# Rhizomatica/mercury

Measured on AMD Instinct MI355X. Metric: RX frames/s (mode 8, max 50 LDPC iters), higher is better.
Workload: dtype f64

## Files before the change

### include/mercury_gpu.h

```cpp
#ifndef MERCURY_GPU_H
#define MERCURY_GPU_H

#include <stddef.h>
#include <stdint.h>

#ifdef __cplusplus
extern "C" {
#endif

#define MGPU_OK 0
#define MGPU_ERR_ARG 1
#define MGPU_ERR_DEVICE 2
#define MGPU_ERR_TABLES 3
#define MGPU_ERR_UNSUPPORTED 4

#define MGPU_DEC_GBF 0
#define MGPU_DEC_SPA 1
#define MGPU_DEC_MINSUM 2
#define MGPU_DEC_SPA_FAST 3

#define MGPU_EST_ZF 0
#define MGPU_EST_LS 1

typedef struct mgpu_ctx mgpu_ctx;
// ... 129 lines not shown
    double avg_iterations;
    long long crc_ok_frames;
} mgpu_error_rate;
int mgpu_baseband_test_esn0(mgpu_ctx* ctx, const double* esn0_db, int npoints, long long frames_per_point, uint64_t seed, uint64_t frame0,
                            int channel, mgpu_error_rate* out);

int mgpu_passband_to_baseband(mgpu_ctx* ctx, const double* passband , int W, int in_size,
                              const double* carrier_hz , int filter, const int* start , int count,
                              int decimation, double* out_c128 );
int mgpu_time_sync_preamble(mgpu_ctx* ctx, const double* baseband_interp_c128 , int W, int size, int step,
                            int location_to_return, int nTrials_max, int* delay , double* correlation );
int mgpu_freq_sync(mgpu_ctx* ctx, const double* baseband_c128 , int W, int stride, double* freq_offset_hz );
int mgpu_time_sync_mfsk(mgpu_ctx* ctx, const double* baseband_interp_c128 , int W, int size, int search_start_symb,
                        int* delay );
int mgpu_detect_ack_pattern(mgpu_ctx* ctx, const double* baseband_interp_c128 , int W, int size, int pattern,
                            double* metric , int* matched );
int mgpu_detect_ack_pattern_from_passband(mgpu_ctx* ctx, const double* passband , int W, int size, double carrier_hz,
                                          int pattern, double* metric , int* matched );
int mgpu_last_sync_kernel_ms(mgpu_ctx* ctx, float* ms);

int mgpu_enable_timing(mgpu_ctx* ctx, int on);
int mgpu_kernel_ms_avg(mgpu_ctx* ctx, float ms[2], int* n_launches);
int mgpu_decoder_hard_frames(mgpu_ctx* ctx, long long* frames);
int mgpu_host_path_last(mgpu_ctx* ctx, int* chunk_frames, int* n_chunks, float* fill_ms, float* drain_ms, float* total_ms);
int mgpu_last_kernel_ms(mgpu_ctx* ctx, float ms[2]);

int mgpu_debug_mfsk_sync(mgpu_ctx* ctx, const double* energy, int W, int nslots, int size, const int* search_start, int variant, int* delay);
int mgpu_debug_p2b_variant(int variant);
int mgpu_debug_span_energy(mgpu_ctx* ctx, const double* bb, int W, int size, const int* wv, const int* off, int n, int len, int variant, double* sum,
                           int* cnt);
int mgpu_debug_spa_math(mgpu_ctx* ctx, const double* in, int n, double* tanh_out, double* atanh_out);
int mgpu_debug_select_peak(mgpu_ctx* ctx, const double* cand_vals, int n, int ncand_max, const int* ncand, const int* size, const int* loc, int step,
                           int nTrials_max, int* delay, double* corr);

int mgpu_debug_occupancy(mgpu_ctx* ctx, int which);

int mgpu_debug_tsync_metric(mgpu_ctx* ctx, const double* baseband_interp, int W, int size, int step, int variant, const int* start, const int* sub_size,
                            double* vals);

int mgpu_debug_glibc_trig(mgpu_ctx* ctx, const double* in, int n, double* atan_out, double* sin_out, double* cos_out);

#ifdef __cplusplus
}
#endif
#endif
```

### mercury_amd/csrc/api.hip

```cpp
#include <hip/hip_runtime.h>

#include <cstdio>
#include <cstdlib>
#include <cstring>
#include <fstream>
#include <algorithm>
#include <atomic>
#include <functional>
#include <stdexcept>
#include <string>
#include <vector>

#include "ctx.hpp"
#include "numa.hpp"

typedef void (*fe_kernel_t)(MgpuDev, const double*, int, float*, float*, float*, double*, MgpuTapsDev);
static fe_kernel_t fe_kernel(int threads) { return threads == 1024 ? mgpu_frontend_kernel_t1024 : mgpu_frontend_kernel; }

thread_local std::string g_create_error;

namespace mgpu_detail {

void ctx_alloc(mgpu_ctx* c) {
    const auto& t = c->tab;
// ... 82 lines not shown
        std::vector<uint8_t> msg(size_t(full > 0 ? full : 1), 0);
        const uint16_t zero = mgpu::crc16_modbus(msg.data(), full);
        std::vector<uint16_t> tab(size_t(full > 0 ? full : 1) * 8, 0);
        for (int b = 0; b < full; ++b)
            for (int j = 0; j < 8; ++j) {
                msg[b] = uint8_t(1u << j);
                tab[size_t(b) * 8 + j] = uint16_t(mgpu::crc16_modbus(msg.data(), full) ^ zero);
                msg[b] = 0;
            }
        l.crc_tab = c->keep(upload(tab));
        l.crc_init = zero;
    }
    l.gdesc = c->keep(upload(t.graph.gdesc));
    l.gkpack = c->keep(upload(t.graph.gkpack));
    l.vinfo_g = c->keep(upload(t.graph.vinfo_g));
    l.Sg = t.graph.Sg;
    l.sadr = c->keep(upload(t.graph.sadr));
    l.bhead = c->keep(upload(t.graph.bhead));
    l.bmask = c->keep(upload(t.graph.bmask));
    l.vinfo2 = c->keep(upload(t.graph.vinfo2));
    l.DM = t.graph.DM;
    l.S = d.S; l.N = d.N; l.P = d.P; l.K = d.K; l.E = d.E; l.nReal = d.nReal; l.payload_stride = d.payload_stride;
    l.max_iters = d.max_iters; l.minsum_alpha = d.minsum_alpha;
    l.hard_frames = reinterpret_cast<unsigned long long*>(c->keep(upload(std::vector<uint64_t>(64, 0))));
    {
        int w[4] = {100, 230, 45, 150};
        if (const char* e = getenv("MERCURY_SPA_SPEC_WEIGHT")) {
            const int n = sscanf(e, "%d,%d,%d,%d", &w[0], &w[1], &w[2], &w[3]);
            if (n == 1) { w[1] = w[2] = w[3] = w[0]; }
            else if (n == 2) { w[2] = w[0]; w[3] = w[1]; }
            else if (n == 3) { w[3] = w[2]; }
        }
        const int nbins = d.S / 64 > 0 ? d.S / 64 : 1;
        auto sample_min = [&](int weight) {
            const long long m = (static_cast<long long>(weight) * 16 + nbins - 1) / nbins;
            return weight <= 0 ? 0 : (m > 0x7fffff ? 0x7fffff : int(m));
        };
        auto byte = [&](int weight) { const int m = sample_min(weight); return unsigned(m > 255 ? 255 : m); };
        l.spec_sample_pack = byte(w[0]) | byte(w[1]) << 8 | byte(w[2]) << 16 | byte(w[3]) << 24;
    }
    HIPCK(hipStreamCreate(&c->stream));
    for (auto& q : c->ev) for (auto& e : q) HIPCK(hipEventCreate(&e));
    for (auto& e : c->sync_ev) HIPCK(hipEventCreate(&e));

    const bool mfsk = t.mfsk_M > 0;
    {
        const char* e = getenv("MERCURY_FE_THREADS");
// ... 8 lines not shown
    {
        int geo[6];
        mgpu_tsync_fine_geometry(geo);
        HIPCK(hipFuncSetAttribute(reinterpret_cast<const void*>(mgpu_tsync_metric_fine_kernel_r4), hipFuncAttributeMaxDynamicSharedMemorySize, geo[2]));
        HIPCK(hipFuncSetAttribute(reinterpret_cast<const void*>(mgpu_tsync_metric_fine_kernel_r8), hipFuncAttributeMaxDynamicSharedMemorySize, geo[5]));
    }
    switch (c->cfg.decoder) {
        case MGPU_DEC_SPA:
            if (!t.graph.fp64_limit.empty()) throw std::runtime_error(t.graph.fp64_limit);
            c->lds_dec = mgpu_spa_lds_bytes(d.S, d.N);
            {
                const int ne = std::max(4, (d.S + 1023) / 1024);
                if (ne > 8) throw std::runtime_error("graph too large for the sum-product kernel");
                if (t.graph.maxdeg > mgpu_spa_max_degree(ne)) throw std::runtime_error("check degree exceeds the sum-product kernel's unrolled product walk");
                switch (ne) {
                    case 4: c->spa_kernel = mgpu_ldpc_spa_kernel_ne4; break;
                    case 5: c->spa_kernel = mgpu_ldpc_spa_kernel_ne5; break;
                    case 6: c->spa_kernel = mgpu_ldpc_spa_kernel_ne6; break;
                    case 7: c->spa_kernel = mgpu_ldpc_spa_kernel_ne7; break;
                    default: c->spa_kernel = mgpu_ldpc_spa_kernel_ne8; break;
                }
            }
            HIPCK(hipFuncSetAttribute(reinterpret_cast<const void*>(c->spa_kernel), hipFuncAttributeMaxDynamicSharedMemorySize, int(c->lds_dec)));
            break;
        case MGPU_DEC_GBF:
            c->lds_dec = mgpu_gbf_lds_bytes(d.N);
            HIPCK(hipFuncSetAttribute(reinterpret_cast<const void*>(mgpu_ldpc_gbf_kernel), hipFuncAttributeMaxDynamicSharedMemorySize, int(c->lds_dec)));
            break;
        case MGPU_DEC_MINSUM: {
            if (!t.graph.fp32_limit.empty()) throw std::runtime_error(t.graph.fp32_limit);
            c->lds_dec = mgpu_spa_fast_lds_bytes(c->ldev.Sg, d.N);
            c->dec_threads = 512;
            c->spa_kernel = mgpu_ldpc_minsum_kernel_t512;
            HIPCK(hipFuncSetAttribute(reinterpret_cast<const void*>(c->spa_kernel), hipFuncAttributeMaxDynamicSharedMemorySize, int(c->lds_dec)));
            break;
        }
        case MGPU_DEC_SPA_FAST: {
            if (!t.graph.fp32_limit.empty()) throw std::runtime_error(t.graph.fp32_limit);
            c->lds_dec = mgpu_spa_fast_lds_bytes(c->ldev.Sg, d.N);
            c->dec_threads = 512;
            c->spa_kernel = mgpu_ldpc_spa_fast_kernel_t512;
            HIPCK(hipFuncSetAttribute(reinterpret_cast<const void*>(c->spa_kernel), hipFuncAttributeMaxDynamicSharedMemorySize, int(c->lds_dec)));
            break;
        }
        default: throw std::runtime_error("unknown decoder");
    }
// ... 429 lines not shown
        out[0] = m.graph.bank_model[0]; out[1] = m.graph.bank_model[1];
        out[2] = m.graph.Sg / 64; out[3] = m.graph.Sg ? double(m.graph.E) / m.graph.Sg : 0;
        return MGPU_OK;
    } catch (const std::exception& e) { g_create_error = e.what(); return MGPU_ERR_ARG; }
}

int mgpu_enable_timing(mgpu_ctx* c, int on) {
    if (!c) return MGPU_ERR_ARG;
    c->timing = on != 0;
    c->ev_count = 0;
    for (auto& b : c->ev_fe) b = false;
    return MGPU_OK;
}

int mgpu_decoder_hard_frames(mgpu_ctx* c, long long* frames) {
    if (!c || !frames) return MGPU_ERR_ARG;
    return guard(c, [&] {
        HIPCK(hipStreamSynchronize(c->stream));
        unsigned long long v[64];
        HIPCK(hipMemcpy(v, c->ldev.hard_frames, sizeof(v), hipMemcpyDeviceToHost));
        long long sum = 0;
        for (unsigned long long x : v) sum += (long long)x;
        *frames = sum;
    });
}

int mgpu_last_kernel_ms(mgpu_ctx* c, float ms[2]) {
    int n = 0;
    return mgpu_kernel_ms_avg(c, ms, &n);
}

int mgpu_kernel_ms_avg(mgpu_ctx* c, float ms[2], int* n_launches) {
    if (!c || !ms) return MGPU_ERR_ARG;
    return guard(c, [&] {
        need(c->timing && c->ev_count > 0, "timing not enabled or nothing launched");
        const int n = c->ev_count < mgpu_ctx::kEvRing ? c->ev_count : mgpu_ctx::kEvRing;
        double fe = 0, dec = 0;
        int nfe = 0;
        for (int i = 0; i < n; ++i) {
            HIPCK(hipEventSynchronize(c->ev[i][3]));
            float t = 0;
            HIPCK(hipEventElapsedTime(&t, c->ev[i][2], c->ev[i][3]));
            dec += t;
            if (c->ev_fe[i]) { HIPCK(hipEventElapsedTime(&t, c->ev[i][0], c->ev[i][1])); fe += t; ++nfe; }
        }
        ms[0] = nfe ? float(fe / nfe) : 0.f;
// ... 733 lines not shown
```

### mercury_amd/csrc/device_tables.h

```cpp
#pragma once
#include <stdint.h>

struct MgpuDev {
    const uint8_t* cell_type;
    const double* pilot_val;
    const uint16_t* pilot_cell;
    const double* constellation;
    const double* twiddle;
    const double* pre_eq;
    const uint16_t* sym_src;
    const uint16_t* llr_src;
    const double* ls_weight;
    const uint8_t* scrambler;
    const uint16_t* llr_dst;
    const uint16_t* bit_il;
    const uint16_t* tf_inv;
    const uint16_t* data_cell;
    const uint32_t* cell_lerp;
    const uint32_t* cptr;
    const uint16_t* cvar;
    int S;
    int M, bps, K, P, N, E;
    int Nsymb, G, nData, nBits, nPilots, nVirtual, nReal;
    int estimator, amp_restore, lsw;
// ... 16 lines not shown
static_assert(double(kSpaHardLlr) - kSpaMaxVarDegree * kSpaClampR >= kSpaTanhSaturates,
              "hard-frame shortcut: |LLR| >= kSpaHardLlr no longer keeps every Q in tanh's saturated range - raise kSpaHardLlr or lower the degree limit");

constexpr uint32_t kSpaOnesBytes = 48 * 8;

struct LdpcDev {
    const uint32_t* cptr; const uint16_t* cvar;
    const uint8_t* scrambler;
    const uint16_t* crc_tab;
    uint32_t crc_init;
    const uint32_t* gdesc; const uint64_t* gkpack; const uint32_t* vinfo_g;
    int Sg;
    const uint32_t* sadr;
    const uint64_t* bhead;
    const uint64_t* bmask;
    const uint32_t* vinfo2;
    int DM;
    int S, N, P, K, E, nReal, payload_stride, max_iters;
    unsigned spec_sample_pack;
    float minsum_alpha;
    unsigned long long* hard_frames;
};

struct MgpuTapsDev {
    double* grid; double* H; double* eq; double* syms; float* llr_demod; double* variance; double* agc_gain;
    long long* cycles;
    double* mean_H;
};

struct MgpuStatsDev {
    int iterations_done, crc, all_zeros, message_decoded;
    float variance, snr_db;
};

struct MgpuMfskSync { int np, nstreams, off[4], tones[8], Nc, sym_period, tail; };
```

### mercury_amd/csrc/ldpc.hip

```cpp
#include <hip/hip_runtime.h>
#include <stdint.h>

#include "device_tables.h"
#ifdef SPA_CENSUS_ON
#include <hip/hip_runtime.h>
__device__ unsigned long long g_spa_census[64];
#define SPA_CENSUS(i) do { const unsigned long long em_ = __builtin_amdgcn_ballot_w64(true); \
    if (int(threadIdx.x & 63) == __builtin_ctzll(em_)) { atomicAdd(&g_spa_census[i], 1ull); atomicAdd(&g_spa_census[32 + (i)], (unsigned long long)__builtin_popcountll(em_)); } } while (0)
extern "C" int mgpu_debug_spa_census(unsigned long long* out, int clear) {
    if (out && hipMemcpyFromSymbol(out, HIP_SYMBOL(g_spa_census), sizeof(g_spa_census)) != hipSuccess) return -1;
    if (clear) { static unsigned long long z[64]; if (hipMemcpyToSymbol(HIP_SYMBOL(g_spa_census), z, sizeof(z)) != hipSuccess) return -1; }
    return 64;
}
#endif
#include "spa_math.h"

#define LDPC_THREADS 1024

#ifdef SPA_STAMPS
#define SPA_STAMP_WGS 8
#define SPA_STAMP_MAX 192
__device__ unsigned long long g_spa_stamps[SPA_STAMP_WGS * 16 * SPA_STAMP_MAX];
#define SPA_STAMP_DECL(F_) int stamp_n = 0; const int stamp_wg = (blockIdx.x % ((F_) / SPA_STAMP_WGS > 0 ? (F_) / SPA_STAMP_WGS : 1)) == ((F_) / (2 * SPA_STAMP_WGS)) ? int(blockIdx.x / ((F_) / SPA_STAMP_WGS > 0 ? (F_) / SPA_STAMP_WGS : 1)) : -1
#define SPA_STAMP(code) do { if (stamp_wg >= 0 && stamp_wg < SPA_STAMP_WGS && (threadIdx.x & 63) == 0 && stamp_n < SPA_STAMP_MAX) { \
    g_spa_stamps[(stamp_wg * 16 + (threadIdx.x >> 6)) * SPA_STAMP_MAX + stamp_n] = (static_cast<unsigned long long>(code) << 56) | (__builtin_amdgcn_s_memrealtime() & 0x00ffffffffffffffull); } ++stamp_n; } while (0)
extern "C" int mgpu_debug_spa_stamps(unsigned long long* out, int clear) {
    if (out && hipMemcpyFromSymbol(out, HIP_SYMBOL(g_spa_stamps), sizeof(g_spa_stamps)) != hipSuccess) return -1;
    if (clear) { static unsigned long long z[SPA_STAMP_WGS * 16 * SPA_STAMP_MAX]; if (hipMemcpyToSymbol(HIP_SYMBOL(g_spa_stamps), z, sizeof(z)) != hipSuccess) return -1; }
    return SPA_STAMP_WGS * 16 * SPA_STAMP_MAX;
}
#else
#define SPA_STAMP_DECL(F_) do {} while (0)
#define SPA_STAMP(code) do {} while (0)
#endif
#ifndef SPA_SPEC_START
#define SPA_SPEC_START 8
#endif
#ifndef SPA_VR_RESIDENT
#define SPA_VR_RESIDENT 1
#endif

namespace {

__device__ void decode_tail(const LdpcDev& T, int f, const uint8_t* hard, uint8_t* bytes_lds, int iterations,
                            uint8_t* __restrict__ bits_out, int* __restrict__ iters_out,
                            uint8_t* __restrict__ payload_out, MgpuStatsDev* __restrict__ stats_out,
                            const float* __restrict__ variance_in, const float* __restrict__ snr_variance_in) {
    const int tid = threadIdx.x;
    if (bits_out) for (int i = tid; i < T.K; i += blockDim.x) bits_out[size_t(f) * T.K + i] = hard[i];
    if (iters_out && tid == 0) iters_out[f] = iterations;
    if (!payload_out && !stats_out) return;
    const int nb = T.nReal, nbytes = (nb + 7) / 8, full = nb / 8;
    unsigned x = 0, nz = 0;
    for (int b = tid; b < nbytes; b += blockDim.x) {
        unsigned v = 0;
        for (int j = 0; j < 8; ++j) {
            const int i = b * 8 + j;
            if (i < nb) v |= unsigned(hard[i] ^ T.scrambler[i]) << j;
        }
        if (payload_out) payload_out[size_t(f) * T.payload_stride + b] = uint8_t(v);
        if (b < full) {
            nz |= v;
// ... 7 lines not shown
    for (int o = 32; o; o >>= 1) x ^= unsigned(__shfl_xor(int(x), o));
    x |= __any(nz != 0) ? 0x10000u : 0u;
    if ((tid & 63) == 0) scratch[tid >> 6] = int(x);
    __syncthreads();
    if (tid == 0) {
        unsigned acc = 0;
        for (int w = 0; w < int(blockDim.x >> 6); ++w) { const unsigned y = unsigned(scratch[w]); acc = ((acc ^ y) & 0xffffu) | ((acc | y) & 0x10000u); }
        const int all_zeros = !(acc & 0x10000u);
        const unsigned crc = all_zeros ? 0u : ((acc & 0xffffu) ^ T.crc_init);
        MgpuStatsDev s;
        s.iterations_done = iterations;
        s.crc = int(crc);
        s.all_zeros = all_zeros;
        s.message_decoded = !(all_zeros || crc != 0);
        s.variance = variance_in ? variance_in[f] : 0.0f;
        const float sv = snr_variance_in ? snr_variance_in[f] : s.variance;
        s.snr_db = s.message_decoded ? float(10.0 * log10(1.0 / double(sv))) : -99.9f;
        stats_out[f] = s;
    }
}

}

extern "C" size_t mgpu_spa_lds_bytes(int S, int N) {
    return size_t(kSpaOnesBytes) + size_t(8) * S + size_t(8) * N + size_t(4) * N + ((N + 15) & ~15) + 256 + 64;
}

constexpr int kN = 1600;

__device__ __forceinline__ void spa_masked_mul2(double& t, double a0, double a1, uint64_t m0, uint64_t m1) {
    uint64_t sv;
    asm volatile(
        "s_and_saveexec_b64 %1, %4\n\t"
        "v_mul_f64 %0, %0, %2\n\t"
        "s_and_b64 exec, %1, %5\n\t"
        "v_mul_f64 %0, %0, %3\n\t"
        "s_mov_b64 exec, %1"
        : "+v"(t), "=&s"(sv)
        : "v"(a0), "v"(a1), "s"(m0), "s"(m1)
        : "scc");
}

typedef uint32_t spa_u32x4 __attribute__((ext_vector_type(4)));
typedef uint32_t spa_u32x2 __attribute__((ext_vector_type(2)));
typedef const uint64_t __attribute__((address_space(4))) * spa_cptr64;
#ifndef SPA_OFF32
#define SPA_OFF32 1
#endif
// ... 17 lines not shown
template <int C, int CMAX>
__device__ __forceinline__ void spa_walk(double& temp, uint32_t achk, spa_cptr64 bm, uint64_t m0, uint64_t m1) {
    typedef __attribute__((address_space(3))) double lds_f64;
    if (m0 == 0) return;
    uint64_t n0 = 0, n1 = 0;
    if constexpr (C + 1 < CMAX) { n0 = bm[2 * C + 2]; n1 = bm[2 * C + 3]; }
    const volatile lds_f64* chk = reinterpret_cast<const volatile lds_f64*>(achk);
    const double a0 = chk[2 * C], a1 = chk[2 * C + 1];
    spa_masked_mul2(temp, a0, a1, m0, m1);
    if constexpr (C + 1 < CMAX) spa_walk<C + 1, CMAX>(temp, achk, bm, n0, n1);
}
template <int C, int CMAX>
__device__ __forceinline__ void spa_walk4(double& temp, uint32_t achk, spa_cptr64 bm, uint64_t m0, uint64_t m1, uint64_t m2, uint64_t m3) {
    typedef __attribute__((address_space(3))) double lds_f64;
    if (m0 == 0) return;
    uint64_t n0 = 0, n1 = 0, n2 = 0, n3 = 0;
    if constexpr (C + 1 < CMAX) { n0 = bm[4 * C + 4]; n1 = bm[4 * C + 5]; n2 = bm[4 * C + 6]; n3 = bm[4 * C + 7]; }
    const volatile lds_f64* chk = reinterpret_cast<const volatile lds_f64*>(achk);
    const double a0 = spa_walk_factor(achk, m0, 4 * C), a1 = spa_walk_factor(achk, m1, 4 * C + 1), a2 = chk[4 * C + 2], a3 = chk[4 * C + 3];
    temp *= a0; SPA_KEEP(temp);
    temp *= a1; SPA_KEEP(temp);
    if (m2 != 0) spa_masked_mul2(temp, a2, a3, m2, m3);
    if constexpr (C + 1 < CMAX) spa_walk4<C + 1, CMAX>(temp, achk, bm, n0, n1, n2, n3);
}

template <int NE, int DMX>
__device__ __forceinline__ void spa_decode(const LdpcDev& T, const float* __restrict__ llr_in, int F,
                                            uint8_t* __restrict__ bits_out, int* __restrict__ iters_out,
                                            uint8_t* __restrict__ payload_out, MgpuStatsDev* __restrict__ stats_out,
                                            const float* __restrict__ variance_in, const float* __restrict__ snr_variance_in) {
    extern __shared__ __attribute__((aligned(16))) unsigned char smem[];
    const int S = T.S;
    constexpr int N = kN;
    constexpr int kMoff = kSpaOnesBytes + N * 8;
    double* Lt = reinterpret_cast<double*>(smem + kSpaOnesBytes);
    double* M = Lt + N;
    float* Li = reinterpret_cast<float*>(M + S);
    uint8_t* hard = reinterpret_cast<uint8_t*>(Li + N);
    uint8_t* bytes = hard + ((N + 15) & ~15);
    int* flag = reinterpret_cast<int*>(bytes + 256);

    const int tid = threadIdx.x, f = blockIdx.x;
    if (f >= F) return;
    if (uint32_t(uintptr_t(smem)) != 0) __builtin_trap();
    if (tid < int(kSpaOnesBytes / 8)) reinterpret_cast<double*>(smem)[tid] = SPA_ALLLANES != 0 && NE != 8 ? 0x1p-10 : 1.0;
    constexpr bool kWaveShortcuts = NE == 8;
    constexpr bool kVaResident = !kWaveShortcuts;
    constexpr bool kAdaptive = !kWaveShortcuts;
    constexpr bool kAllLanes = SPA_ALLLANES != 0 && (!kWaveShortcuts || SPA_ALLLANES8 != 0);
    constexpr int kSpecStart = SPA_SPEC_START;
    SPA_STAMP_DECL(F);
    SPA_STAMP(1);
    const float* lin = llr_in + size_t(f) * N;
    int hard_lane = 1;
    for (int v = tid; v < N; v += LDPC_THREADS) {
        const float l = lin[v];
        Li[v] = l;
        Lt[v] = spa_tanh_half(double(l));
        hard_lane &= int(__builtin_fabsf(l) >= kSpaHardLlr);
    }
    const int wave = __builtin_amdgcn_readfirstlane(tid >> 6);
    struct VarRec { uint32_t vi, w0, w1, w2, w3, w4; };
    const __amdgpu_buffer_rsrc_t vrec = __builtin_amdgcn_make_buffer_rsrc(const_cast<uint32_t*>(T.vinfo2), 0, N * 32, 0x00020000);
    auto load_var = [&](int i) -> VarRec {
        const spa_u32x4 lo = __builtin_amdgcn_raw_buffer_load_b128(vrec, i * 32, 0, 0);
        const spa_u32x2 hi = __builtin_amdgcn_raw_buffer_load_b64(vrec, i * 32, 16, 0);
        return VarRec{lo.x, lo.y, lo.z, lo.w, hi.x, hi.y};
    };
    typedef __attribute__((address_space(3))) double lds_f64;
    auto ldsd = [](uint32_t byte_off) -> lds_f64* { return reinterpret_cast<lds_f64*>(byte_off); };
    auto Mb = [&](uint32_t byte_off) -> double { return *ldsd(kMoff + byte_off); };
    auto var_update = [&](const VarRec& q) {
        const uint32_t v = q.vi & 0x7ff;
        uint32_t deg = q.vi >> 11;
        asm volatile("" : "+v"(deg));
        double s = Li[v];
        if (deg > 0) { s += Mb(q.w0 & 0xffff); SPA_KEEP(s); }
        if (deg > 1) { s += Mb(q.w0 >> 16); SPA_KEEP(s); }
        if (deg > 2) {
            s += Mb(q.w1 & 0xffff); SPA_KEEP(s);
            if (deg > 3) { s += Mb(q.w1 >> 16); SPA_KEEP(s); }
            if (deg > 4) { s += Mb(q.w2 & 0xffff); SPA_KEEP(s); }
            if (deg > 5) {
                s += Mb(q.w2 >> 16); SPA_KEEP(s);
                if (deg > 6) { s += Mb(q.w3 & 0xffff); SPA_KEEP(s); }
                if (deg > 7) { s += Mb(q.w3 >> 16); SPA_KEEP(s); }
                if (deg > 8) { s += Mb(q.w4 & 0xffff); SPA_KEEP(s); }
            }
        }
        Lt[v] = s;
    };
    auto var_update4 = [&](uint32_t vi, uint32_t w0, uint32_t w1) {
        const uint32_t v = vi & 0x7ff;
        uint32_t deg = vi >> 11;
        asm volatile("" : "+v"(deg));
        double s = Li[v];
        if (deg > 0) { s += Mb(w0 & 0xffff); SPA_KEEP(s); }
        if (deg > 1) { s += Mb(w0 >> 16); SPA_KEEP(s); }
        if (deg > 2) {
            s += Mb(w1 & 0xffff); SPA_KEEP(s);
            if (deg > 3) { s += Mb(w1 >> 16); SPA_KEEP(s); }
        }
        Lt[v] = s;
    };
    if (tid == 0) { flag[0] = 0; flag[1] = 0; flag[2] = LDPC_THREADS / 64; flag[3] = LDPC_THREADS / 64; }
    int* hard_w = reinterpret_cast<int*>(bytes);
    const int hard_wave = __builtin_amdgcn_ballot_w64(hard_lane == 0) == 0;
    if ((tid & 63) == 0) hard_w[tid >> 6] = hard_wave;
    __syncthreads();
    const bool hard_frame = __builtin_amdgcn_ballot_w64((tid & 63) < LDPC_THREADS / 64 && hard_w[tid & 15] == 0) == 0;

    auto bin_prefix = [&](unsigned long long m, unsigned long long ends) -> unsigned long long {
        m ^= m << 1; m ^= m << 2; m ^= m << 4; m ^= m << 8; m ^= m << 16; m ^= m << 32;
        return m & ends;
    };
    auto bin_unsat = [&](unsigned long long m, unsigned long long ends) -> bool { return bin_prefix(m, ends) != 0; };
    auto bin_odd_count = [&](unsigned long long pre, unsigned long long used, unsigned long long ends) -> int {
        return __builtin_popcountll(pre ^ (((pre << 1) + (used & ~ends)) & ends));
    };
    auto flag_report = [&](int p, bool unsat, int cnt) {
        if (unsat && (tid & 63) == 0) __hip_atomic_fetch_add(&flag[p & 1], 1 + (cnt << 8), __ATOMIC_RELAXED, __HIP_MEMORY_SCOPE_WORKGROUP);
    };
    const __amdgpu_buffer_rsrc_t sadr = __builtin_amdgcn_make_buffer_rsrc(const_cast<uint32_t*>(T.sadr), 0, 0x7fffffff, 0x00020000);
    constexpr int kRound = LDPC_THREADS * 8;
    const spa_cptr64 bhead0 = (spa_cptr64)(T.bhead) + size_t(wave) * 4;

    struct SynPre { uint32_t alt[NE]; unsigned long long vmask[NE], ends[NE]; };
    auto syn_fetch = [&](SynPre& q) {
// ... 72 lines not shown
                if constexpr (kWaveShortcuts) rr = spa_atanh_x2_wave(temp, kAllLanes ? lanes_in_use : ~0ull);
                else rr = spa_atanh_x2(temp);
            }
            __builtin_amdgcn_wave_barrier();
            if (kAllLanes || valid) *ldsd(own) = rr;
            b = nxt;
        }
        if (with_syndrome && unsat && (tid & 63) == 0) flag[p & 1] = 1;
    };
#if SPA_VR_RESIDENT
    VarRec va;
    if constexpr (kVaResident) va = load_var(tid);
    spa_u32x4 vb;
#endif
    int iteration = 0;
    SPA_STAMP(2);
    syndrome_pass(0);
    SPA_STAMP(3);
    __syncthreads();
    SPA_STAMP(4);
    int look = flag[0];
    if (look && hard_frame) {
        iteration = T.max_iters + 1;
        if (tid == 0 && T.hard_frames) atomicAdd(T.hard_frames + (f & 63), 1ull);
    }
    else if (look) {
        auto run_after = [&](int lk, int shift) -> int {
            const int n = lk >> 8, one = int(T.spec_sample_pack >> shift) & 255, two = int(T.spec_sample_pack >> (shift + 8)) & 255;
            return !kAdaptive ? 0 : (n >= two && two != 255) ? 2 : (n >= one && one != 255) ? 1 : 0;
        };
        constexpr int kCtlSpec = 1 << 16, kCtlRun = 1 << 20;
        int ctl = 1 + kCtlRun * run_after(look, 0);
        for (;; ++ctl) {
            asm volatile("" : "+s"(ctl));
            const int it = ctl & 0xffff;
            const bool spec = (ctl & kCtlSpec) != 0;
            const bool skip = it >= kSpecStart || ctl >= kCtlRun;
            if (it == 1) cn_pass(false, 0, std::true_type());
            else if (it <= T.max_iters) cn_pass((ctl & kCtlSpec) != 0, it - 1, std::false_type());
            else syndrome_pass(it - 1);
            asm volatile("" : "+s"(ctl));
#if !SPA_VR_RESIDENT
            const VarRec va = load_var(tid), vb = load_var(tid + LDPC_THREADS);
#else
            if constexpr (!kVaResident) va = load_var(tid);
            vb = __builtin_amdgcn_raw_buffer_load_b128(vrec, (tid + LDPC_THREADS) * 32, 0, 0);
#endif
            SPA_STAMP(5);
            __syncthreads();
            SPA_STAMP(6);
            if (spec) {
                look = flag[(it - 1) & 1];
                if (!look) { iteration = it - 1; break; }
                if (it > T.max_iters) { iteration = T.max_iters + 1; break; }
            }
            if (tid == 0) { flag[it & 1] = 0; flag[2 + (it & 1)] = LDPC_THREADS / 64; }
            SynPre pre;
            if (!skip) syn_fetch(pre);
#if SPA_VR_RESIDENT
            VarRec qa = va;
            spa_u32x4 qb = vb;
            asm volatile("" : "+v"(qa.vi), "+v"(qa.w0), "+v"(qa.w1), "+v"(qa.w2), "+v"(qa.w3), "+v"(qa.w4), "+v"(qb));
            var_update(qa);
            if (tid + LDPC_THREADS < N) var_update4(qb.x, qb.y, qb.z);
#else
            var_update(va);
            if (tid + LDPC_THREADS < N) var_update(vb);
#endif
            if (!skip) syn_pin(pre);
            SPA_STAMP(7);
            __syncthreads();
            SPA_STAMP(8);
            ctl = skip ? (ctl | kCtlSpec) - (ctl >= kCtlRun ? kCtlRun : 0) : ctl & ~kCtlSpec;
            if (!skip) {
                syn_judge(pre, it);
                SPA_STAMP(3);
                __syncthreads();
                SPA_STAMP(4);
                look = flag[it & 1];
                if (!look) { iteration = it; break; }
                if (it == T.max_iters) { iteration = T.max_iters + 1; break; }
                ctl += kCtlRun * run_after(look, 16);
            }
        }
    }
    SPA_STAMP(9);
    for (int v = tid; v < N; v += LDPC_THREADS) hard[v] = Lt[v] < 0;
    __syncthreads();
    decode_tail(T, f, hard, bytes, iteration, bits_out, iters_out, payload_out, stats_out, variance_in, snr_variance_in);
    SPA_STAMP(10);
}

#define SPA_KERNEL(NE, DMX)                                                                                    \
    extern "C" __global__ __launch_bounds__(LDPC_THREADS, 8) void mgpu_ldpc_spa_kernel_ne##NE(               \
        LdpcDev T, const float* __restrict__ llr_in, int F, uint8_t* __restrict__ bits_out,                     \
        int* __restrict__ iters_out, uint8_t* __restrict__ payload_out, MgpuStatsDev* __restrict__ stats_out,   \
        const float* __restrict__ variance_in, const float* __restrict__ snr_variance_in) {                     \
        spa_decode<NE, DMX>(T, llr_in, F, bits_out, iters_out, payload_out, stats_out, variance_in, snr_variance_in); \
    }
SPA_KERNEL(4, 16)
SPA_KERNEL(5, 16)
SPA_KERNEL(6, 16)
SPA_KERNEL(7, 16)
SPA_KERNEL(8, 48)
extern "C" int mgpu_spa_max_degree(int ne) { return ne == 8 ? 48 : 16; }

template <int CTRL>
// ... 291 lines not shown
```

### mercury_amd/physical_layer.py

```python
import ctypes as C
import os

import numpy as np

HERE = os.path.dirname(os.path.abspath(__file__))
LIB_PATH = os.environ.get("MERCURY_GPU_LIB") or os.path.join(HERE, "libmercury_gpu.so")

DEC_GBF, DEC_SPA, DEC_MINSUM, DEC_SPA_FAST = 0, 1, 2, 3
EST_ZF, EST_LS = 0, 1


class Config(C.Structure):
    _fields_ = [("cfg", C.c_int), ("max_iters", C.c_int), ("decoder", C.c_int), ("agc", C.c_int),
                ("variance_source", C.c_int), ("device", C.c_int), ("max_batch", C.c_int),
                ("minsum_alpha", C.c_float), ("mfsk_ctrl_mode", C.c_int), ("test_puncture_nBits", C.c_int)]


INFO_FIELDS = ("cfg M bits_per_symbol K P N Nsymb Nc Nfft Ngi Nofdm nData nBits nPilots nVirtual nReal "
               "bit_blk tf_blk preamble_nsymb estimator amp_restore ls_window Cwidth Vwidth E "
               "payload_bytes payload_stride frame_samples mfsk_M mfsk_nStreams active_nsymb active_nbits").split()


class ExplicitParams(C.Structure):
    _fields_ = [("pilot_boost", C.c_float), ("ls_window", C.c_int), ("seeds_set", C.c_int), ("pilot_seed", C.c_uint),
# ... 48 lines not shown
            pass
        lib = C.CDLL(LIB_PATH)
        lib.mgpu_last_error.restype = C.c_char_p
        lib.mgpu_last_error.argtypes = [C.c_void_p]
        lib.mgpu_create.argtypes = [C.POINTER(Config), C.POINTER(C.c_void_p)]
        lib.mgpu_txgen_dev.argtypes = [C.c_void_p, C.c_uint64, C.c_uint64, C.c_int, C.c_double, C.c_int,
                                       C.c_void_p, C.c_void_p, C.c_void_p]
        lib.mgpu_rx_batch_dev.argtypes = [C.c_void_p, C.c_void_p, C.c_int, C.c_void_p, C.c_void_p, C.c_void_p, C.c_void_p]
        lib.mgpu_frontend_dev.argtypes = [C.c_void_p, C.c_void_p, C.c_int, C.c_void_p, C.c_void_p, C.c_void_p]
        lib.mgpu_ldpc_batch_dev.argtypes = [C.c_void_p, C.c_void_p, C.c_int, C.c_void_p, C.c_void_p, C.c_void_p,
                                            C.c_void_p, C.c_void_p, C.c_void_p]
        lib.mgpu_destroy.argtypes = [C.c_void_p]
        _lib = lib
    return _lib


EXPORTED_SYMBOLS = [
    "mgpu_alloc_host", "mgpu_free_host", "mgpu_create", "mgpu_destroy", "mgpu_last_error", "mgpu_get_info", "mgpu_rx_batch", "mgpu_rx_batch_taps",
    "mgpu_host_libm_selfcheck", "mgpu_host_select_peak", "mgpu_host_fir_taps", "mgpu_host_preamble_carriers", "mgpu_host_mode_info", "mgpu_host_layout_stats",
    "mgpu_device_props_get", "mgpu_alloc_host_near", "mgpu_host_numa_node_of_pci", "mgpu_host_numa_cpus", "mgpu_pool_device_numa_node",
    "mgpu_ldpc_batch", "mgpu_ldpc_encode_batch", "mgpu_rx_batch_dev", "mgpu_frontend_dev", "mgpu_ldpc_batch_dev", "mgpu_txgen_dev",
    "mgpu_host_path_last", "mgpu_device_malloc", "mgpu_device_free", "mgpu_context_stream", "mgpu_synchronize", "mgpu_copy_to_host", "mgpu_copy_to_device",
    "mgpu_pool_rx_batch_dev", "mgpu_pool_ldpc_batch_dev", "mgpu_pool_txgen_dev",
    "mgpu_last_kernel_ms", "mgpu_kernel_ms_avg", "mgpu_decoder_hard_frames", "mgpu_enable_timing", "mgpu_debug_spa_math", "mgpu_debug_glibc_trig", "mgpu_debug_tsync_metric", "mgpu_debug_occupancy", "mgpu_debug_select_peak", "mgpu_debug_span_energy", "mgpu_debug_p2b_variant", "mgpu_debug_mfsk_sync", "mgpu_baseband_test_esn0", "mgpu_passband_test_esn0", "mgpu_passband_to_baseband", "mgpu_time_sync_preamble", "mgpu_freq_sync", "mgpu_last_sync_kernel_ms",
    "mgpu_time_sync_mfsk", "mgpu_detect_ack_pattern", "mgpu_detect_ack_pattern_from_passband",
    "mgpu_receive_buffer_nsymb", "mgpu_receive_byte_batch", "mgpu_receive_byte_batch_samples", "mgpu_measure_signal_only",
    "mgpu_host_pre_equalization_channel", "mgpu_context_pre_equalization_channel", "mgpu_set_pre_equalization_channel", "mgpu_transmit_bit_batch", "mgpu_transmit_frame_samples", "mgpu_transmit_byte_batch", "mgpu_transmit_byte_batch_dev", "mgpu_transmit_buffer", "mgpu_symbol_mod", "mgpu_generate_ack_pattern_passband",
    "mgpu_symbol_demod", "mgpu_automatic_gain_control", "mgpu_channel_estimator", "mgpu_restore_channel_amplitude", "mgpu_channel_equalizer",
    "mgpu_measure_variance", "mgpu_deframer", "mgpu_deinterleaver_c128", "mgpu_deinterleaver_f32", "mgpu_psk_demod",
    "mgpu_bit_energy_dispersal", "mgpu_bit_to_byte", "mgpu_crc16_modbus_rtu",
    "mgpu_shm_create", "mgpu_shm_connect", "mgpu_shm_close", "mgpu_shm_destroy", "mgpu_shm_used", "mgpu_shm_free", "mgpu_shm_capacity",
    "mgpu_shm_clear", "mgpu_shm_write", "mgpu_shm_read", "mgpu_shm_read_all", "mgpu_shm_publish_decoded",
    "mgpu_create_explicit", "mgpu_pool_create", "mgpu_pool_destroy", "mgpu_pool_size", "mgpu_pool_context", "mgpu_pool_last_error", "mgpu_pool_last_counters",
    "mgpu_pool_shard", "mgpu_pool_rx_batch", "mgpu_pool_ldpc_batch", "mgpu_pool_receive_byte_batch",
]


def cfg_explicit(M, rate16, preamble_nsymb, estimator):
    mods, rates = {2: 0, 4: 1, 8: 2, 16: 3, 32: 4}, {1: 0, 2: 1, 3: 2, 4: 3, 5: 4, 6: 5, 8: 6, 14: 7}
    if M not in mods or rate16 not in rates or not 1 <= preamble_nsymb <= 8 or estimator not in (0, 1):
        return -1
    return 1000 + (((mods[M] * 8 + rates[rate16]) * 8 + (preamble_nsymb - 1)) * 2 + estimator)


class MgpuError(RuntimeError):
    pass

# ... 383 lines not shown
        return a, s, c

    def debug_spa_math(self, x):
        xin = np.ascontiguousarray(x, np.float64).ravel()
        t = np.zeros_like(xin)
        a = np.zeros_like(xin)
        self._ck(self.lib.mgpu_debug_spa_math(self.h, _ptr(xin), C.c_int(xin.size), _ptr(t), _ptr(a)))
        return t, a

    def enable_timing(self, on=True):
        self._ck(self.lib.mgpu_enable_timing(self.h, C.c_int(1 if on else 0)))

    def host_path_last(self):
        a, b = C.c_int(), C.c_int()
        f, d, t = C.c_float(), C.c_float(), C.c_float()
        self._ck(self.lib.mgpu_host_path_last(self.h, C.byref(a), C.byref(b), C.byref(f), C.byref(d), C.byref(t)))
        return {"chunk_frames": a.value, "n_chunks": b.value, "fill_ms": f.value, "drain_ms": d.value, "total_ms": t.value}

    def decoder_hard_frames(self):
        n = C.c_longlong(0)
        self._ck(self.lib.mgpu_decoder_hard_frames(self.h, C.byref(n)))
        return int(n.value)

    def kernel_ms_avg(self):
        ms = (C.c_float * 2)()
        n = C.c_int(0)
        self._ck(self.lib.mgpu_kernel_ms_avg(self.h, ms, C.byref(n)))
        return float(ms[0]), float(ms[1]), int(n.value)


POOL_MAX_DEVICES = 16


class ErrorRate(C.Structure):
    _fields_ = [("esn0_db", C.c_double), ("Frames_total", C.c_longlong), ("Error_frames_total", C.c_longlong), ("Bits_total", C.c_longlong),
                ("Error_bits_total", C.c_longlong), ("BER", C.c_double), ("FER", C.c_double), ("avg_iterations", C.c_double),
                ("crc_ok_frames", C.c_longlong)]


class PoolCounters(C.Structure):
    _fields_ = [("n_devices", C.c_int), ("frames", C.c_longlong), ("decoded", C.c_longlong), ("ldpc_iterations", C.c_longlong),
                ("wall_ms", C.c_double), ("device_frames", C.c_int * POOL_MAX_DEVICES), ("device_ms", C.c_double * POOL_MAX_DEVICES)]


def pool_shard(F, G, g):
    lib = load_library()
# ... 161 lines not shown
```

Baseline: 734,700.

## Detect periodic SPA decoder cycles and skip remaining iterations

After a threshold iteration, each iteration's variable-node totals are hashed through DPP lane XORs and LDS atomics into a ring of per-iteration hashes. When the current hash matches an earlier one, the check-to-variable message array is snapshotted into a global pool slot. If the messages match the snapshot exactly one period later, the decoder jumps ahead by whole periods or exits early, since a non-converging decoder stuck in a limit cycle would only repeat the same states up to max_iters. This saves iterations on frames that never converge, at the cost of hashing work every iteration, extra LDS, global atomics for slot allocation, and snapshot copies. It also adds a counter of executed iterations.

Result: no change. 735,500, median of 6 (+0.1%).

```diff
diff --git a/include/mercury_gpu.h b/include/mercury_gpu.h
--- a/include/mercury_gpu.h
+++ b/include/mercury_gpu.h
@@ -175,6 +175,7 @@
 int mgpu_enable_timing(mgpu_ctx* ctx, int on);
 int mgpu_kernel_ms_avg(mgpu_ctx* ctx, float ms[2], int* n_launches);
 int mgpu_decoder_hard_frames(mgpu_ctx* ctx, long long* frames);
+int mgpu_decoder_executed_iterations(mgpu_ctx* ctx, long long* iterations);
 int mgpu_host_path_last(mgpu_ctx* ctx, int* chunk_frames, int* n_chunks, float* fill_ms, float* drain_ms, float* total_ms);
 int mgpu_last_kernel_ms(mgpu_ctx* ctx, float ms[2]);
 
diff --git a/mercury_amd/csrc/api.hip b/mercury_amd/csrc/api.hip
--- a/mercury_amd/csrc/api.hip
+++ b/mercury_amd/csrc/api.hip
@@ -128,7 +128,7 @@
     l.DM = t.graph.DM;
     l.S = d.S; l.N = d.N; l.P = d.P; l.K = d.K; l.E = d.E; l.nReal = d.nReal; l.payload_stride = d.payload_stride;
     l.max_iters = d.max_iters; l.minsum_alpha = d.minsum_alpha;
-    l.hard_frames = reinterpret_cast<unsigned long long*>(c->keep(upload(std::vector<uint64_t>(64, 0))));
+    l.hard_frames = reinterpret_cast<unsigned long long*>(c->keep(upload(std::vector<uint64_t>(sizeof(SpaCounters) / 8, 0))));
     {
         int w[4] = {100, 230, 45, 150};
         if (const char* e = getenv("MERCURY_SPA_SPEC_WEIGHT")) {
@@ -183,6 +183,20 @@
                 }
             }
             HIPCK(hipFuncSetAttribute(reinterpret_cast<const void*>(c->spa_kernel), hipFuncAttributeMaxDynamicSharedMemorySize, int(c->lds_dec)));
+            if (const char* e = getenv("MERCURY_SPA_CYCLE"); !(e && atoi(e) == 0)) {
+                int per_cu = 0;
+                HIPCK(hipOccupancyMaxActiveBlocksPerMultiprocessor(&per_cu, c->spa_kernel, c->dec_threads, c->lds_dec));
+                hipDeviceProp_t p;
+                HIPCK(hipGetDeviceProperties(&p, c->cfg.device));
+                const int slots = (std::max(1, per_cu) * std::max(1, p.multiProcessorCount) + 31) & ~31;
+                double* pool = nullptr;
+                HIPCK(hipMalloc(&pool, sizeof(double) * size_t(slots) * size_t(d.S)));
+                SpaCounters cnt{};
+                cnt.cycle_pool = c->keep(pool);
+                cnt.cycle_map = c->keep(upload(std::vector<uint32_t>(size_t(slots / 32), 0u)));
+                cnt.cycle_slots = slots;
+                HIPCK(hipMemcpy(reinterpret_cast<SpaCounters*>(l.hard_frames), &cnt, sizeof(cnt), hipMemcpyHostToDevice));
+            }
             break;
         case MGPU_DEC_GBF:
             c->lds_dec = mgpu_gbf_lds_bytes(d.N);
@@ -658,6 +672,18 @@
         long long sum = 0;
         for (unsigned long long x : v) sum += (long long)x;
         *frames = sum;
+    });
+}
+
+int mgpu_decoder_executed_iterations(mgpu_ctx* c, long long* iterations) {
+    if (!c || !iterations) return MGPU_ERR_ARG;
+    return guard(c, [&] {
+        HIPCK(hipStreamSynchronize(c->stream));
+        unsigned long long v[64];
+        HIPCK(hipMemcpy(v, reinterpret_cast<SpaCounters*>(c->ldev.hard_frames)->exec_iters, sizeof(v), hipMemcpyDeviceToHost));
+        long long sum = 0;
+        for (unsigned long long x : v) sum += (long long)x;
+        *iterations = sum;
     });
 }
 
diff --git a/mercury_amd/csrc/device_tables.h b/mercury_amd/csrc/device_tables.h
--- a/mercury_amd/csrc/device_tables.h
+++ b/mercury_amd/csrc/device_tables.h
@@ -62,6 +62,14 @@
     unsigned long long* hard_frames;
 };
 
+struct SpaCounters {
+    unsigned long long hard_frames[64];
+    unsigned long long exec_iters[64];
+    double* cycle_pool;
+    unsigned* cycle_map;
+    long long cycle_slots;
+};
+
 struct MgpuTapsDev {
     double* grid; double* H; double* eq; double* syms; float* llr_demod; double* variance; double* agc_gain;
     long long* cycles;
diff --git a/mercury_amd/csrc/ldpc.hip b/mercury_amd/csrc/ldpc.hip
--- a/mercury_amd/csrc/ldpc.hip
+++ b/mercury_amd/csrc/ldpc.hip
@@ -38,6 +38,18 @@
 #endif
 #ifndef SPA_VR_RESIDENT
 #define SPA_VR_RESIDENT 1
+#endif
+#ifndef SPA_CYCLE
+#define SPA_CYCLE 1
+#endif
+#ifndef SPA_CYCLE_LOWRATES
+#define SPA_CYCLE_LOWRATES 0
+#endif
+#ifndef SPA_CYCLE_FROM
+#define SPA_CYCLE_FROM 24
+#endif
+#ifndef SPA_CYCLE_FROM8
+#define SPA_CYCLE_FROM8 2
 #endif
 
 namespace {
@@ -91,8 +103,11 @@
 
 }
 
+constexpr int kCycleRing = 32;
+constexpr int kCycleHist = kCycleRing - 2;
+constexpr int kCycleState = 8;
 extern "C" size_t mgpu_spa_lds_bytes(int S, int N) {
-    return size_t(kSpaOnesBytes) + size_t(8) * S + size_t(8) * N + size_t(4) * N + ((N + 15) & ~15) + 256 + 64;
+    return size_t(kSpaOnesBytes) + size_t(8) * S + size_t(8) * N + size_t(4) * N + ((N + 15) & ~15) + 256 + 64 + 4 * (kCycleRing + kCycleState);
 }
 
 constexpr int kN = 1600;
@@ -156,6 +171,19 @@
     temp *= a1; SPA_KEEP(temp);
     if (m2 != 0) spa_masked_mul2(temp, a2, a3, m2, m3);
     if constexpr (C + 1 < CMAX) spa_walk4<C + 1, CMAX>(temp, achk, bm, n0, n1, n2, n3);
+}
+
+__device__ __forceinline__ uint32_t spa_cycle_fold(double s, uint32_t v) {
+    const uint32_t x = uint32_t(__double2loint(s)) ^ uint32_t(__double2hiint(s));
+    return __builtin_amdgcn_alignbit(x, x, v);
+}
+__device__ __forceinline__ void spa_cycle_publish(uint32_t h, uint32_t* word, int tid) {
+    auto x = [](uint32_t a, auto ctrl) { return a ^ uint32_t(__builtin_amdgcn_update_dpp(0, int(a), decltype(ctrl)::value, 0xf, 0xf, false)); };
+    h = x(h, std::integral_constant<int, 0xb1>());
+    h = x(h, std::integral_constant<int, 0x4e>());
+    h = x(h, std::integral_constant<int, 0x141>());
+    h = x(h, std::integral_constant<int, 0x140>());
+    if ((tid & 15) == 0) __hip_atomic_fetch_xor(word, h, __ATOMIC_RELAXED, __HIP_MEMORY_SCOPE_WORKGROUP);
 }
 
 template <int NE, int DMX>
@@ -173,6 +201,8 @@
     uint8_t* hard = reinterpret_cast<uint8_t*>(Li + N);
     uint8_t* bytes = hard + ((N + 15) & ~15);
     int* flag = reinterpret_cast<int*>(bytes + 256);
+    uint32_t* cyh = reinterpret_cast<uint32_t*>(bytes + 256 + 64);
+    int* cys = reinterpret_cast<int*>(cyh + kCycleRing);
 
     const int tid = threadIdx.x, f = blockIdx.x;
     if (f >= F) return;
@@ -183,6 +213,8 @@
     constexpr bool kAdaptive = !kWaveShortcuts;
     constexpr bool kAllLanes = SPA_ALLLANES != 0 && (!kWaveShortcuts || SPA_ALLLANES8 != 0);
     constexpr int kSpecStart = SPA_SPEC_START;
+    constexpr bool kCycle = SPA_CYCLE != 0 && (kWaveShortcuts || SPA_CYCLE_LOWRATES != 0);
+    constexpr int kCycleFrom = kWaveShortcuts ? SPA_CYCLE_FROM8 : SPA_CYCLE_FROM;
     SPA_STAMP_DECL(F);
     SPA_STAMP(1);
     const float* lin = llr_in + size_t(f) * N;
@@ -223,6 +255,7 @@
             }
         }
         Lt[v] = s;
+        return spa_cycle_fold(s, v);
     };
     auto var_update4 = [&](uint32_t vi, uint32_t w0, uint32_t w1) {
         const uint32_t v = vi & 0x7ff;
@@ -236,8 +269,15 @@
             if (deg > 3) { s += Mb(w1 >> 16); SPA_KEEP(s); }
         }
         Lt[v] = s;
-    };
-    if (tid == 0) { flag[0] = 0; flag[1] = 0; flag[2] = LDPC_THREADS / 64; flag[3] = LDPC_THREADS / 64; }
+        return spa_cycle_fold(s, v);
+    };
+    if (tid == 0) {
+        flag[0] = 0; flag[1] = 0; flag[2] = LDPC_THREADS / 64; flag[3] = LDPC_THREADS / 64;
+        const SpaCounters* sc = reinterpret_cast<const SpaCounters*>(T.hard_frames);
+        cys[0] = kCycle && sc->cycle_pool ? 1 : 0; cys[4] = 0;
+        const uint64_t a = uint64_t(uintptr_t(sc));
+        cys[6] = int(uint32_t(a)); cys[7] = int(uint32_t(a >> 32));
+    }
     int* hard_w = reinterpret_cast<int*>(bytes);
     const int hard_wave = __builtin_amdgcn_ballot_w64(hard_lane == 0) == 0;
     if ((tid & 63) == 0) hard_w[tid >> 6] = hard_wave;
@@ -356,7 +396,8 @@
     int look = flag[0];
     if (look && hard_frame) {
         iteration = T.max_iters + 1;
-        if (tid == 0 && T.hard_frames) atomicAdd(T.hard_frames + (f & 63), 1ull);
+        if (tid == 0) atomicAdd(T.hard_frames + (f & 63), 1ull);
+        if (tid == 0) cys[4] = T.max_iters;
     }
     else if (look) {
         auto run_after = [&](int lk, int shift) -> int {
@@ -388,19 +429,21 @@
                 if (!look) { iteration = it - 1; break; }
                 if (it > T.max_iters) { iteration = T.max_iters + 1; break; }
             }
-            if (tid == 0) { flag[it & 1] = 0; flag[2 + (it & 1)] = LDPC_THREADS / 64; }
+            if (tid == 0) { flag[it & 1] = 0; flag[2 + (it & 1)] = LDPC_THREADS / 64; cyh[(it + 1) & (kCycleRing - 1)] = 0; }
+            const bool hash_on = kCycle && it >= kCycleFrom && __builtin_amdgcn_readfirstlane(cys[0]) != 0;
             SynPre pre;
             if (!skip) syn_fetch(pre);
 #if SPA_VR_RESIDENT
             VarRec qa = va;
             spa_u32x4 qb = vb;
             asm volatile("" : "+v"(qa.vi), "+v"(qa.w0), "+v"(qa.w1), "+v"(qa.w2), "+v"(qa.w3), "+v"(qa.w4), "+v"(qb));
-            var_update(qa);
-            if (tid + LDPC_THREADS < N) var_update4(qb.x, qb.y, qb.z);
+            uint32_t hv = var_update(qa);
+            if (tid + LDPC_THREADS < N) hv ^= var_update4(qb.x, qb.y, qb.z);
 #else
-            var_update(va);
-            if (tid + LDPC_THREADS < N) var_update(vb);
-#endif
+            uint32_t hv = var_update(va);
+            if (tid + LDPC_THREADS < N) hv ^= var_update(vb);
+#endif
+            if (hash_on) spa_cycle_publish(hv, &cyh[it & (kCycleRing - 1)], tid);
             if (!skip) syn_pin(pre);
             SPA_STAMP(7);
             __syncthreads();
@@ -416,7 +459,70 @@
                 if (it == T.max_iters) { iteration = T.max_iters + 1; break; }
                 ctl += kCtlRun * run_after(look, 16);
             }
-        }
+            if (kCycle && it >= kCycleFrom && it < T.max_iters) {
+                const int mode = __builtin_amdgcn_readfirstlane(cys[0]);
+                SpaCounters* sc = reinterpret_cast<SpaCounters*>(uintptr_t(uint32_t(__builtin_amdgcn_readfirstlane(cys[6])))
+                                                                 | uintptr_t(uint32_t(__builtin_amdgcn_readfirstlane(cys[7]))) << 32);
+                const uint64_t* Mu = reinterpret_cast<const uint64_t*>(M);
+                if (mode == 2 && it == __builtin_amdgcn_readfirstlane(cys[2] + cys[3])) {
+                    const int slot = __builtin_amdgcn_readfirstlane(cys[1]), p = __builtin_amdgcn_readfirstlane(cys[3]);
+                    const uint64_t* snap = reinterpret_cast<const uint64_t*>(sc->cycle_pool) + size_t(slot) * S;
+                    bool diff = false;
+                    for (int e = tid; e < S; e += LDPC_THREADS) diff |= Mu[e] != snap[e];
+                    if (__ballot(diff) != 0 && (tid & 63) == 0) cys[5] = 1;
+                    if (tid == 0) { flag[(it + 1) & 1] = 0; flag[2 + ((it + 1) & 1)] = LDPC_THREADS / 64; }
+                    __syncthreads();
+                    const bool same = __builtin_amdgcn_readfirstlane(cys[5]) == 0;
+                    if (tid == 0) {
+                        __threadfence();
+                        atomicAnd(sc->cycle_map + (slot >> 5), ~(1u << (slot & 31)));
+                        cys[0] = same ? 0 : 1;
+                    }
+                    if (same) {
+                        const int skip_n = (T.max_iters - it) / p * p;
+                        if (tid == 0) cys[4] = skip_n;
+                        if (skip_n == T.max_iters - it) { iteration = T.max_iters + 1; break; }
+                        ctl += skip_n;
+                    }
+                } else if (mode == 1) {
+                    const int j = tid & 63;
+                    const uint32_t h0 = cyh[it & (kCycleRing - 1)];
+                    const bool hit = j >= 1 && j <= kCycleHist && it - j >= kCycleFrom && cyh[(it - j) & (kCycleRing - 1)] == h0;
+                    const uint64_t m = __ballot(hit);
+                    if (m != 0) {
+                        if (tid == 0) {
+                            int got = -1;
+                            const int nw = int(sc->cycle_slots >> 5);
+                            const int w0 = int(h0 % unsigned(nw));
+                            for (int k = 0; k < nw && got < 0; ++k) {
+                                const int w = (w0 + k) % nw;
+                                unsigned cur = __hip_atomic_load(sc->cycle_map + w, __ATOMIC_RELAXED, __HIP_MEMORY_SCOPE_AGENT);
+                                while (cur != ~0u) {
+                                    const int b = __builtin_ctz(~cur);
+                                    const unsigned old = atomicOr(sc->cycle_map + w, 1u << b);
+                                    if (!(old & (1u << b))) { got = w * 32 + b; break; }
+                                    cur = old;
+                                }
+                            }
+                            cys[1] = got; cys[2] = it; cys[3] = __builtin_ctzll(m); cys[5] = 0;
+                        }
+                        __syncthreads();
+                        const int slot = __builtin_amdgcn_readfirstlane(cys[1]);
+                        if (slot >= 0) {
+                            if (tid == 0) cys[0] = 2;
+                            uint64_t* snap = reinterpret_cast<uint64_t*>(sc->cycle_pool) + size_t(slot) * S;
+                            for (int e = tid; e < S; e += LDPC_THREADS) snap[e] = Mu[e];
+                            __syncthreads();
+                        }
+                    }
+                }
+            }
+        }
+    }
+    if (tid == 0) {
+        SpaCounters* sc = reinterpret_cast<SpaCounters*>(T.hard_frames);
+        if (kCycle && cys[0] == 2) { __threadfence(); atomicAnd(sc->cycle_map + (cys[1] >> 5), ~(1u << (cys[1] & 31))); }
+        atomicAdd(sc->exec_iters + (f & 63), (unsigned long long)((iteration > T.max_iters ? T.max_iters : iteration) - cys[4]));
     }
     SPA_STAMP(9);
     for (int v = tid; v < N; v += LDPC_THREADS) hard[v] = Lt[v] < 0;
diff --git a/mercury_amd/physical_layer.py b/mercury_amd/physical_layer.py
--- a/mercury_amd/physical_layer.py
+++ b/mercury_amd/physical_layer.py
@@ -94,7 +94,7 @@
     "mgpu_ldpc_batch", "mgpu_ldpc_encode_batch", "mgpu_rx_batch_dev", "mgpu_frontend_dev", "mgpu_ldpc_batch_dev", "mgpu_txgen_dev",
     "mgpu_host_path_last", "mgpu_device_malloc", "mgpu_device_free", "mgpu_context_stream", "mgpu_synchronize", "mgpu_copy_to_host", "mgpu_copy_to_device",
     "mgpu_pool_rx_batch_dev", "mgpu_pool_ldpc_batch_dev", "mgpu_pool_txgen_dev",
-    "mgpu_last_kernel_ms", "mgpu_kernel_ms_avg", "mgpu_decoder_hard_frames", "mgpu_enable_timing", "mgpu_debug_spa_math", "mgpu_debug_glibc_trig", "mgpu_debug_tsync_metric", "mgpu_debug_occupancy", "mgpu_debug_select_peak", "mgpu_debug_span_energy", "mgpu_debug_p2b_variant", "mgpu_debug_mfsk_sync", "mgpu_baseband_test_esn0", "mgpu_passband_test_esn0", "mgpu_passband_to_baseband", "mgpu_time_sync_preamble", "mgpu_freq_sync", "mgpu_last_sync_kernel_ms",
+    "mgpu_last_kernel_ms", "mgpu_kernel_ms_avg", "mgpu_decoder_hard_frames", "mgpu_decoder_executed_iterations", "mgpu_enable_timing", "mgpu_debug_spa_math", "mgpu_debug_glibc_trig", "mgpu_debug_tsync_metric", "mgpu_debug_occupancy", "mgpu_debug_select_peak", "mgpu_debug_span_energy", "mgpu_debug_p2b_variant", "mgpu_debug_mfsk_sync", "mgpu_baseband_test_esn0", "mgpu_passband_test_esn0", "mgpu_passband_to_baseband", "mgpu_time_sync_preamble", "mgpu_freq_sync", "mgpu_last_sync_kernel_ms",
     "mgpu_time_sync_mfsk", "mgpu_detect_ack_pattern", "mgpu_detect_ack_pattern_from_passband",
     "mgpu_receive_buffer_nsymb", "mgpu_receive_byte_batch", "mgpu_receive_byte_batch_samples", "mgpu_measure_signal_only",
     "mgpu_host_pre_equalization_channel", "mgpu_context_pre_equalization_channel", "mgpu_set_pre_equalization_channel", "mgpu_transmit_bit_batch", "mgpu_transmit_frame_samples", "mgpu_transmit_byte_batch", "mgpu_transmit_byte_batch_dev", "mgpu_transmit_buffer", "mgpu_symbol_mod", "mgpu_generate_ack_pattern_passband",
@@ -524,6 +524,11 @@
         self._ck(self.lib.mgpu_decoder_hard_frames(self.h, C.byref(n)))
         return int(n.value)
 
+    def decoder_executed_iterations(self):
+        n = C.c_longlong(0)
+        self._ck(self.lib.mgpu_decoder_executed_iterations(self.h, C.byref(n)))
+        return int(n.value)
+
     def kernel_ms_avg(self):
         ms = (C.c_float * 2)()
         n = C.c_int(0)
```
